# jketterl/digiham

Hardware: AMD Instinct MI355X
Metric: concurrent 48 kS/s DMR channels sustained end-to-end (rrc_filter->gfsk_demodulator->dmr_decoder) (higher is better)
Workload: dtype f32; 1 GPU; 16384 DMR channels/GPU x 3.96 s (190080 samples) of 48 kS/s FM-discriminator audio, full chain rrc(wide)->gfsk(10)->dmr_decoder incl. BPTC(196,96) (BASELINE con; channels_per_gpu=16384, total_channels=16384

## Files before the change

digiham_amd/csrc/dsp_core.hpp:

```cpp
#pragma once

#include "dh_portable.hpp"
#include "wave_ops.hpp"

#define DH_VARIANCE_SYMBOLS 100
#define DH_VOLUME_RB_SIZE 100
#define DH_FTILE 1024
#define DH_FIR_L 16
#define DH_PF_N 5
#define DH_PF_SINK 512
#define DH_MAX_NZ 160
#define DH_MAX_SPS 40
DH_HD uint32_t dh_history(uint32_t sps) { return DH_VARIANCE_SYMBOLS * (sps > 10u ? sps : 10u) + 152u; }
DH_HD uint32_t dh_tail_max(uint32_t sps) { return 256u + dh_history(sps); }
#define DH_STATE_HDR 32

enum { DH_ST_K = 0, DH_ST_OFF = 1, DH_ST_TAIL = 2, DH_ST_NSYM = 3, DH_ST_ORDERED = 4, DH_ST_BLOCKS = 5,
       DH_ST_P0 = 6,
       DH_ST_CUR_START = 7, DH_ST_CUR_OFF = 8, DH_ST_PREV_START = 9, DH_ST_PREV_OFF = 10,
       DH_ST_BLOCK_FLAGS = 11,
       DH_ST_E_CUR = 12, DH_ST_E_PREV = 13, DH_ST_E_COUNT = 14, DH_ST_E_BLOCK = 15,
       DH_ST_UNCERTAIN = 16, DH_ST_EXACT_RUNS = 17, DH_ST_EXACT_BLOCKS = 18,
       DH_ST_PART = 19,
       DH_ST_DIAG = 20 };
// ... 297 lines not shown
        float acc = 0.0f;
        for (int p = 0; p < NZ + 16; p++) acc = __builtin_fmaf(xs[DH_XPAD(b16 + (uint32_t) p)], tapsf[p - n], acc);
        acc16[4 * T + r] = acc;
    }
}
#endif

#define DH_EXACT_BATCH 2
#define DH_F16_KSTEPS_OF(nz) (((nz) + 16 + 31) / 32)
#define DH_F16_MAX_KSTEPS DH_F16_KSTEPS_OF(DH_MAX_NZ)
#define DH_F16_HALVES_OF(nz) (1008 + 32 * DH_F16_KSTEPS_OF(nz))
#define DH_F16_H2_OFFSET_OF(nz) (DH_F16_HALVES_OF(nz) / 2)
#define DH_F16_ROW_BLOCK(m) (2u * ((uint32_t) (m) & 3u) + (((uint32_t) (m) >> 2) & 1u) + 8u * ((uint32_t) (m) >> 3))
#define DH_F16_OUT(T, r, g, n) (256u * (uint32_t) (T) + 128u * ((uint32_t) (g) >> 1) + 32u * (uint32_t) (r) + 16u * ((uint32_t) (g) & 1u) + (uint32_t) (n))

struct DhF16Taps {
    uint32_t frag[2 * DH_F16_MAX_KSTEPS][DH_WAVE][4];
    uint32_t ksteps;
    double l1, l1_g1, l1_g2, sum_delta;
};
inline void dh_f16_tap_fragments(const float* taps_half, uint32_t nz, DhF16Taps& F) {
    uint16_t g1[DH_MAX_NZ + 1], g2[DH_MAX_NZ + 1];
    F.l1 = F.l1_g1 = F.l1_g2 = F.sum_delta = 0.0;
    for (uint32_t i = 0; i <= nz; i++) {
        const float c = taps_half[i <= nz / 2 ? i : nz - i];
        g1[i] = dh_f16_bits(c);
        const double r = (double) c - (double) dh_f16_value(g1[i]);
        g2[i] = dh_f16_bits((float) (r * 2048.0));
        const double v2 = (double) dh_f16_value(g2[i]);
        const double delta = r - v2 / 2048.0;
        F.l1 += c < 0 ? -(double) c : (double) c; F.l1_g1 += __builtin_fabs((double) dh_f16_value(g1[i]));
        F.l1_g2 += __builtin_fabs(v2); F.sum_delta += __builtin_fabs(delta);
    }
    const int KS = (int) DH_F16_KSTEPS_OF(nz);
    F.ksteps = (uint32_t) KS;
    for (int f = 0; f < 2 * KS; f++) for (int lane = 0; lane < DH_WAVE; lane++) for (int d = 0; d < 4; d++) {
        const int n = lane & 15, q = lane >> 4, s = f % KS;
        uint32_t w = 0;
        for (int hh = 0; hh < 2; hh++) {
            const int t = 32 * s + 8 * q + 2 * d + hh - n;
            const uint16_t v = (t >= 0 && t <= (int) nz) ? (f < KS ? g1[t] : g2[t]) : 0;
            w |= (uint32_t) v << (16 * hh);
        }
        F.frag[f][lane][d] = w;
    }
}
inline float dh_f16_error_coefficient(const DhF16Taps& F, uint32_t nz, double gain) {
    const double u = 5.9604644775390625e-08;
    const double ks = (double) F.ksteps, nref = 2.0 + (double) nz;
    const double kl1 = (nref + 0.01) * F.l1 + 1.0001 * F.l1 + 41.0 * ks * F.l1_g1 * (1.0 + 1.0 / 2048.0) + 82.0 * ks / 2048.0 * (F.l1_g2 + 0.5 * F.l1_g1)
                     + 2.0 * (0.5 * F.l1_g2 / 4194304.0 + F.sum_delta * (1.0 + 1.0 / 4096.0) + u * F.l1) / u + 3.1 * F.l1;
    const double coef = 1.44 * kl1 * u / (gain < 0 ? -gain : gain) * 1.0001;
    float f = (float) coef;
    if ((double) f < coef) { union { float f; uint32_t u; } b; b.f = f; b.u++; f = b.f; }
    return f;
}

#if DH_ON_GPU
template <int NZ>
__device__ __forceinline__ void dh_fir_f16(const float* hw, const dh_u4 (&G)[2 * DH_F16_KSTEPS_OF(NZ)], int lane, float k1, float k2, float* out16) {
    constexpr int DH_F16_KSTEPS = DH_F16_KSTEPS_OF(NZ), DH_F16_FRAGS = 2 * DH_F16_KSTEPS, DH_F16_H2_OFFSET = DH_F16_H2_OFFSET_OF(NZ);
    const int m = lane & 15, q = lane >> 4;
    const char* base = reinterpret_cast<const char*>(hw) + 32 * (int) DH_F16_ROW_BLOCK(m) + 16 * q;
    dh_h8 g[DH_F16_FRAGS];
#pragma unroll
    for (int f = 0; f < DH_F16_FRAGS; f++) g[f] = __builtin_bit_cast(dh_h8, G[f]);
#pragma unroll
    for (int TT = 0; TT < 4; TT += 2) {
        dh_h8 a1[2][DH_F16_KSTEPS], a2[2][DH_F16_KSTEPS];
#pragma unroll
        for (int t = 0; t < 2; t++)
#pragma unroll
            for (int s = 0; s < DH_F16_KSTEPS; s++) a1[t][s] = *reinterpret_cast<const dh_h8*>(base + 512 * (TT + t) + 64 * s);
        dh_f32x4 mn[2] = { { 0.0f, 0.0f, 0.0f, 0.0f }, { 0.0f, 0.0f, 0.0f, 0.0f } }, sc[2] = { { 0.0f, 0.0f, 0.0f, 0.0f }, { 0.0f, 0.0f, 0.0f, 0.0f } };
#pragma unroll
        for (int s = 0; s < DH_F16_KSTEPS; s++) {
#pragma unroll
            for (int t = 0; t < 2; t++) sc[t] = __builtin_amdgcn_mfma_f32_16x16x32_f16(a1[t][s], g[DH_F16_KSTEPS + s], sc[t], 0, 0, 0);
#pragma unroll
            for (int t = 0; t < 2; t++) mn[t] = __builtin_amdgcn_mfma_f32_16x16x32_f16(a1[t][s], g[s], mn[t], 0, 0, 0);
#pragma unroll
            for (int t = 0; t < 2; t++) a2[t][s] = *reinterpret_cast<const dh_h8*>(base + 512 * (TT + t) + 64 * s + 4 * DH_F16_H2_OFFSET);
        }
#pragma unroll
        for (int s = 0; s < DH_F16_KSTEPS; s++)
#pragma unroll
            for (int t = 0; t < 2; t++) sc[t] = __builtin_amdgcn_mfma_f32_16x16x32_f16(a2[t][s], g[s], sc[t], 0, 0, 0);
#pragma unroll
        for (int t = 0; t < 2; t++)
#pragma unroll
            for (int r = 0; r < 4; r++) out16[4 * (TT + t) + r] = __builtin_fmaf(sc[t][r], k2, mn[t][r] * k1);
        __builtin_amdgcn_sched_group_barrier(0x100, 2 * DH_F16_KSTEPS, 0);
#pragma unroll
        for (int s = 0; s < DH_F16_KSTEPS; s++) { __builtin_amdgcn_sched_group_barrier(0x008, 4, 0); __builtin_amdgcn_sched_group_barrier(0x100, 2, 0); }
        __builtin_amdgcn_sched_group_barrier(0x008, 2 * DH_F16_KSTEPS, 0);
    }
}
#else
template <int NZ>
inline void dh_fir_f16(const float* hw, const uint32_t (*G)[DH_WAVE][4], int lane, float k1, float k2, float* out16) {
    constexpr int DH_F16_KSTEPS = DH_F16_KSTEPS_OF(NZ), DH_F16_H2_OFFSET = DH_F16_H2_OFFSET_OF(NZ);
    const uint16_t* h1 = reinterpret_cast<const uint16_t*>(hw);
    const uint16_t* h2 = reinterpret_cast<const uint16_t*>(hw + DH_F16_H2_OFFSET);
    const int n = lane & 15, g = lane >> 4;
    for (int T = 0; T < 4; T++) for (int r = 0; r < 4; r++) {
        const uint32_t o = DH_F16_OUT(T, r, g, n), b16 = o - (uint32_t) n;
        float mn = 0.0f, sc = 0.0f;
        for (int pass = 0; pass < 3; pass++)
            for (int s = 0; s < DH_F16_KSTEPS; s++) for (int qq = 0; qq < 4; qq++) for (int j = 0; j < 8; j++) {
                const int kk = 8 * qq + j;
                const uint32_t w = G[(pass == 1 ? DH_F16_KSTEPS : 0) + s][16 * qq + n][j >> 1];
                const float tap = dh_f16_value((uint16_t) (w >> (16 * (j & 1))));
                const uint16_t hv = (pass == 2 ? h2 : h1)[b16 + 32u * (uint32_t) s + (uint32_t) kk];
                if (pass == 0) mn = __builtin_fmaf(dh_f16_value(hv), tap, mn); else sc = __builtin_fmaf(dh_f16_value(hv), tap, sc);
            }
        out16[4 * T + r] = __builtin_fmaf(sc, k2, mn * k1);
    }
}
#endif

DH_HD float dh_virtual_sample(const float* tail, uint32_t tc, const float* in, uint32_t idx) {
    return idx < tc ? tail[idx] : in[idx - tc];
}

struct DhAgcPair { float mn0, mx0, mn1, mx1; };

#if DH_ON_GPU
__device__ __forceinline__ void dh_agc_scan(DhDspShared& S, uint32_t k0, uint32_t k1, DH_LANE_STRUCT_REF(DhAgcPair, agc)) {
    const int lane = dh_fresh_lane_id_();
    const uint32_t e0 = 2u * (uint32_t) lane, e1 = e0 + 1u;
    const float c0 = e0 < k0 ? S.vol_old[e0] : S.vol_new[e0];
// ... 754 lines not shown
}
template <int NZ> struct DhWindowGroups {
    static constexpr uint32_t GSTEP = NZ > 0 ? DH_XPAD(4u * DH_WAVE) : 4u * DH_WAVE;
    static constexpr uint32_t LAST_LANES = (DH_FTILE + NZ - 4u * DH_WAVE * (DH_PF_N - 1)) / 4u;
    static constexpr uint32_t STORE_LANES = (DH_F16_HALVES_OF(NZ) - 4u * DH_WAVE * (DH_PF_N - 1)) / 4u;
    static_assert((DH_FTILE + NZ) % 4u == 0 && (DH_FTILE + NZ) >= 4u * DH_WAVE * (DH_PF_N - 1) && LAST_LANES <= DH_WAVE, "four full groups + a partial one cover the window");
    static_assert(STORE_LANES >= LAST_LANES && STORE_LANES <= DH_WAVE, "the partial group covers the padded arrays");
};
#define DH_STORE_FIR_OUT(xf, lane, fo) do { \
        dh_f4a* dst_ = reinterpret_cast<dh_f4a*>((xf) + DH_FIR_L * (lane)); \
        _Pragma("unroll") for (int j_ = 0; j_ < DH_FIR_L / 4; j_++) { \
            dh_f4a v_; v_.x = DH_LA(fo, lane)[4 * j_]; v_.y = DH_LA(fo, lane)[4 * j_ + 1]; \
            v_.z = DH_LA(fo, lane)[4 * j_ + 2]; v_.w = DH_LA(fo, lane)[4 * j_ + 3]; \
            dst_[j_] = v_; \
        } } while (0)
template <int NZ>
DH_HD bool dh_stage_f16(const DhDspParams& P, DhDspShared& S, DH_LANE_ARRAY(dh_f4, (&varr), DH_PF_N), uint32_t have, float& e_out, float& k1_out, float& k2_out) {
    constexpr uint32_t LAST_LANES = DhWindowGroups<NZ>::LAST_LANES, STORE_LANES = DhWindowGroups<NZ>::STORE_LANES;
    DH_LANE_ARRAY(float, xm, 1);
    DH_FOR_LANES_FRESH(lane) {
        const uint32_t l4 = 4u * (uint32_t) lane;
        if (DH_UNLIKELY(have < DH_FTILE + NZ)) {
#pragma unroll
            for (int r = 0; r < DH_PF_N; r++) {
                const uint32_t e = l4 + 4u * DH_WAVE * (uint32_t) r;
                DH_LA(varr, lane)[r] = dh_zero_beyond(DH_LA(varr, lane)[r], e, have);
            }
        }
        const float mx = dh_max_abs_groups(DH_LA(varr, lane));
        DH_LA(xm, lane)[0] = mx;
    }
    const float xmax = DH_WAVE_MAX(xm);
    float scale = 1.0f;
    if (xmax == 0.0f) { e_out = 0.0f; k1_out = P.inv_gain; }
    else if (xmax >= DH_BOUND_XMAX_LO && xmax <= DH_BOUND_XMAX_HI) {
        union { float f; uint32_t u; } b; b.f = xmax;
        const uint32_t ex = b.u >> 23;
        b.u = (253u - ex) << 23; scale = b.f;
        b.u = (ex + 1u) << 23; k1_out = P.inv_gain * b.f;
        e_out = P.err_coef_f16 * xmax;
    } else return false;
    k2_out = k1_out * 0.00048828125f;
    DH_FOR_LANES_FRESH(lane) {
        const bool in_last = (uint32_t) lane < LAST_LANES, in_store = (uint32_t) lane < STORE_LANES;
        if (STORE_LANES > LAST_LANES && !in_last) { dh_f4 z; z.x = 0.0f; z.y = 0.0f; z.z = 0.0f; z.w = 0.0f; DH_LA(varr, lane)[DH_PF_N - 1] = z; }
        dh_h4* d1 = reinterpret_cast<dh_h4*>(S.xf) + lane;
        dh_h4* d2 = reinterpret_cast<dh_h4*>(S.xf + DH_F16_H2_OFFSET_OF(NZ)) + lane;
#pragma unroll
        for (int r = 0; r < DH_PF_N; r++) {
            dh_h4 a, b;
            dh_f16_split4(DH_LA(varr, lane)[r], scale, a, b);
            if (r < DH_PF_N - 1 || in_store) { dh_h4_store(d1 + DH_WAVE * r, a); dh_h4_store(d2 + DH_WAVE * r, b); }
        }
    }
    return true;
}

template <int NZ, bool PF_REG>
DH_HD void dh_issue_next_window(DhDspShared& S, const float* const& in, const uint32_t& tc, const uint32_t& p_next, const bool& pf_plain, const bool& pf_reg, DH_LANE_ARRAY(dh_f4, (&pfr), PF_REG ? DH_PF_N : 1)) {
    (void) S; (void) pfr;
    if (DH_LIKELY(pf_reg)) {
        constexpr uint32_t LAST_LANES = DhWindowGroups<NZ>::LAST_LANES;
        const float* src = in + (p_next - tc);
        DH_FOR_LANES_FRESH(lane) {
            const float* lsrc = src + 4u * (uint32_t) lane;
            const bool in_last = (uint32_t) lane < LAST_LANES;
// ... 3 lines not shown
            else (void) in_last;
        }
    } else {
        if (pf_plain) dh_l2_touch_lines(in + (p_next - tc), DH_FTILE + NZ, S.xf + DH_PF_SINK);
    }
}

#define DH_TAIL_GROUPS 8
#define DH_RING_GROUPS 16

template <int NZ, bool FAST, int SPS, int LV = 0, int KEEPF = 0>
DH_HD void dh_rrc_demod_channel(const DhDspParams& P, uint32_t ch, DhDspShared& S, uint32_t part_lo = 0, uint32_t part_hi = 0xFFFFFFFFu, uint32_t sym_base = 0) {
    static_assert(SPS == 0 || SPS == 10 || SPS == 20 || SPS == 40, "0 = run-time samples per symbol; 10 has its own window and timing code, 20 / 40 are the generic code with the constant folded in");
    constexpr bool BOUNDED = DhIsBounded<NZ, FAST, SPS>::value;
    constexpr bool MF16 = BOUNDED && (NZ == 80 || NZ == 160) && KEEPF != 2;
    DhBoundState* const BS = DH_BOUND_STATE(S);
    float* st = P.state + (size_t) ch * P.state_stride;
    uint32_t* sth = (uint32_t*) st;
    const uint32_t sps = SPS ? (uint32_t) SPS : P.sps;
    const uint32_t ev_lo = SPS == 10 ? 3u : SPS == 20 ? 7u : SPS == 40 ? 13u : P.lo, ev_hi = SPS == 10 ? 7u : SPS == 20 ? 13u : SPS == 40 ? 27u : P.hi;
    const float sps_rcp = 1.0f / (float) sps;
    float* tail = st + DH_ST_VAR + DH_VARIANCE_SYMBOLS * sps;
    const float* in = P.in + (size_t) ch * P.in_stride + part_lo;
    uint8_t* syms = P.syms + (size_t) ch * P.sym_stride;
    const float* in_end = P.in + (size_t) (P.n_channels - 1u) * P.in_stride + P.n;
    const ptrdiff_t in_room = (in_end - in) - (ptrdiff_t) (DH_FTILE + NZ);
    const uint32_t win_lim = dh_uniform(in_room < 0 ? 0u : in_room >= (ptrdiff_t) 0xFFFFFFFFu ? 0xFFFFFFFFu : (uint32_t) in_room + 1u);

    DH_PHASE_MARK_BEGIN();
    uint32_t k0 = sth[DH_ST_K];
// ... 147 lines not shown
                        }
                    }
                    if (BOUNDED) {
                        float mx = 0.0f;
#pragma unroll
                        for (int r = 0; r < DH_PF_N; r++) {
                            const dh_f4 w = DH_LA(v, lane)[r];
                            mx = dh_max3_abs(w.x, w.y, mx); mx = dh_max3_abs(w.z, w.w, mx);
                        }
                        DH_LA(xmax_lane, lane)[0] = mx;
                    }
                }
            }
            if (MF16 && !use_exact) {
                xmax_done = true;
                if (dh_stage_f16<NZ>(P, S, v, have, e_run, k1, k2)) f16_staged = true; else use_exact = true;
            }
            if (!f16_staged) {
                DH_FOR_LANES_FRESH(lane) {
                    const uint32_t l4 = 4u * (uint32_t) lane;
                    const bool in_last = (uint32_t) lane < LAST_LANES;
                    float* ldst = &S.xf[DH_XP(l4)];
                    dh_lds_store4_at<0>(ldst, DH_LA(v, lane)[0]); dh_lds_store4_at<GSTEP>(ldst, DH_LA(v, lane)[1]);
                    dh_lds_store4_at<2 * GSTEP>(ldst, DH_LA(v, lane)[2]); dh_lds_store4_at<3 * GSTEP>(ldst, DH_LA(v, lane)[3]);
                    static_assert(DH_PF_N == 5, "four full groups + a partial one");
                    if constexpr (LAST_LANES > 0) { if (in_last) dh_lds_store4_at<4 * GSTEP>(ldst, DH_LA(v, lane)[4]); }
                    dh_lds_stores_done();
                }
            }
        } else if (MF16 && !use_exact) {
            const uint32_t have = dh_min<uint32_t>(DH_FTILE + NZ, nv - p);
            DH_LANE_ARRAY(dh_f4, v, DH_PF_N);
            DH_FOR_LANES_FRESH(lane) {
#pragma unroll
                for (int r = 0; r < DH_PF_N; r++) {
                    const uint32_t e = 4u * (uint32_t) lane + 4u * DH_WAVE * (uint32_t) r;
                    dh_f4 w;
                    w.x = e + 0u < have ? dh_virtual_sample(tail, tc, in, p + e + 0u) : 0.0f;
                    w.y = e + 1u < have ? dh_virtual_sample(tail, tc, in, p + e + 1u) : 0.0f;
                    w.z = e + 2u < have ? dh_virtual_sample(tail, tc, in, p + e + 2u) : 0.0f;
                    w.w = e + 3u < have ? dh_virtual_sample(tail, tc, in, p + e + 3u) : 0.0f;
                    DH_LA(v, lane)[r] = w;
                }
            }
            xmax_done = true;
            if (dh_stage_f16<NZ>(P, S, v, have, e_run, k1, k2)) f16_staged = true;
            else {
                use_exact = true;
                dh_gather_window<NZ>(S, tail, tc, in, nv, p);
            }
        } else if (p >= tc) {
            use_exact = BOUNDED;
            const float* src = in + (p - tc);
            const uint32_t have = dh_min<uint32_t>(DH_FTILE + NZ, nv - p);
            DH_FOR_LANES_FRESH(lane) {
                for (uint32_t e = 4u * (uint32_t) lane; e < DH_FTILE + NZ; e += 4u * DH_WAVE) {
                    dh_f4 v;
                    if (e + 4u <= have) v = dh_load4_unaligned(src + e);
                    else {
                        v.x = e + 0u < have ? src[e + 0u] : 0.0f; v.y = e + 1u < have ? src[e + 1u] : 0.0f;
                        v.z = e + 2u < have ? src[e + 2u] : 0.0f; v.w = e + 3u < have ? src[e + 3u] : 0.0f;
                    }
                    dh_store4(&S.xf[DH_XP(e)], v);
                }
            }
        } else {
            use_exact = BOUNDED;
            dh_gather_window<NZ>(S, tail, tc, in, nv, p);
        }
        DH_BARRIER();
        if (BOUNDED && !use_exact && !xmax_done) {
            const float xmax = DH_WAVE_MAX(xmax_lane);
            if (xmax == 0.0f) e_run = 0.0f;
            else if (xmax >= DH_BOUND_XMAX_LO && xmax <= DH_BOUND_XMAX_HI) e_run = P.err_coef * xmax;
            else use_exact = true;
        }
        DH_PHASE_MARK(0);

        if (NZ > 0 && DH_STOP_AFTER >= 2) {
            DH_LANE_ARRAY(float, fo, DH_FIR_L);
            DH_COMPILER_FENCE();
            constexpr bool MFMA = NZ > 0 && NZ <= 80 && (BOUNDED || FAST) && !MF16;
            int mf_layout = 0;
            if (BOUNDED) {
                uint64_t vote_bad = 0;
                if (DH_LIKELY(!use_exact)) {
                    if constexpr (MF16) {
                        DH_FOR_LANES_FRESH(lane) {
                            float t = 0.0f;
                            dh_fir_f16<MF16 ? NZ : 80>(S.xf, tapfrag_regs, lane, k1, k2, DH_LA(fo, lane));
#pragma unroll
                            for (int j = 0; j < DH_FIR_L; j++) t = __builtin_fmaf(DH_LA(fo, lane)[j], 0.0f, t);
                            DH_BALLOT_ACC(vote_bad, !(t == 0.0f), lane);
                        }
                        mf_layout = 2;
                    } else if constexpr (MFMA) {
                        DH_FOR_LANES_FRESH(lane) {
                            bool bad = false;
                            float acc[DH_FIR_L];
                            dh_fir_mfma<MFMA ? NZ : 80>(S.tapsf, S.xf, lane, acc);
                            dh_fir_finish<true>(acc, P.gain, P.rgain, P.inv_gain, DH_LA(fo, lane), &bad);
                            DH_BALLOT_ACC(vote_bad, bad, lane);
                        }
                        mf_layout = 1;
                    } else static_assert(!BOUNDED, "every error-bounded kernel filters on the matrix cores (launch_plan.hpp instantiates none without MF16 or MFMA)");
                }
                if (DH_UNLIKELY(use_exact || vote_bad)) {
                    use_exact = true; e_run = 0.0f; BS->n_exact_runs++; mf_layout = 0;
// ... 101 lines not shown
        const bool block_done = (k0 + m == DH_VARIANCE_SYMBOLS);
        if (block_done && DH_STOP_AFTER >= 6) {
            new_off = dh_timing_decision<NZ, SPS, BOUNDED>(P, S, BS, V, sps, k0, e_blk);
        }

        DH_PHASE_MARK(5);
        DH_FOR_LANES_FRESH(lane) {
            const uint32_t ka = k0 + (uint32_t) lane, kb = ka + DH_WAVE, ke = k0 + m;
            const uint32_t ia = ka < ke ? ka : k0, ib = kb < ke ? kb : k0;
            const float va_ = S.vol_new[ia], vb_ = S.vol_new[ib];
            S.vol_old[ia] = va_;
            S.vol_old[ib] = vb_;
        }
        staged_p = 0xFFFFFFFFu;
        if (DH_LIKELY(pf_reg)) {
            if constexpr (PF_REG && MF16) { if (DH_LIKELY(dh_stage_f16<NZ>(P, S, pfr, pf_have, st_e_run, st_k1, st_k2))) staged_p = p_next; }
            else if constexpr (PF_PLAIN) {
                static_assert(!PF_PLAIN || (DH_FTILE == 4u * DH_WAVE * (DH_PF_N - 1)), "four full groups cover the window");
                DH_FOR_LANES_FRESH(lane) {
                    const uint32_t l4 = 4u * (uint32_t) lane;
                    float* ldst = &S.xf[l4];
#pragma unroll
                    for (int r = 0; r < DH_PF_N - 1; r++) {
                        dh_f4 w = DH_LA(pfr, lane)[PF_REG ? r : 0];
                        if (DH_UNLIKELY(pf_have < DH_FTILE)) w = dh_zero_beyond(w, l4 + 4u * DH_WAVE * (uint32_t) r, pf_have);
                        dh_store4(ldst + 4 * DH_WAVE * r, w);
                    }
                }
                staged_p = p_next;
            }
        }
// ... 180 lines not shown
```

digiham_amd/csrc/engine_impl.hpp:

```cpp
#pragma once

#include <stdlib.h>
#include <string.h>
#include <new>
#include <vector>

#include "../../include/digiham_amd.h"
#include "dsp_core.hpp"
#include "decoder_core.hpp"
#include "kernels_core.hpp"
#include "fec_tables.hpp"
#include "rrc_taps.h"

namespace dh {

struct Layout {
    uint32_t B, max_samples, sps, nz, lo, hi;
    int rrc, demod, proto;
    uint32_t flags;
    uint32_t sym_cap, out_cap, ev_cap;
    size_t sym_stride, state_words;
    bool fused;
    int fused_keep;
};
// ... 129 lines not shown
        if (!ok) return DH_ENOMEM;
        configure(c.rrc_gain);
        if (L.proto) {
            DhFecTables* host = new (std::nothrow) DhFecTables;
            if (!host) return DH_ENOMEM;
            build_fec_tables(*host);
            rc = be.upload(tables, host, sizeof(DhFecTables));
            be.sync();
            delete host;
            if (rc) return rc;
        }
        if (L.rrc == DH_RRC_CUSTOM && (be.upload(custom_taps, c.rrc_taps, sizeof(float) * (L.nz + 1)) || be.sync())) return DH_EDEVICE;
        if (tapfrag) {
            DhF16Taps* F = new (std::nothrow) DhF16Taps;
            if (!F) return DH_ENOMEM;
            dh_f16_tap_fragments(dsp.taps, L.nz, *F);
            dsp.err_coef_f16 = dh_f16_error_coefficient(*F, L.nz, dsp.gain);
            rc = be.upload(tapfrag, F->frag, sizeof(F->frag)) || be.sync();
            delete F;
            if (rc) return DH_EDEVICE;
        }
        return reset();
    }

    void configure(double custom_gain) {
        fast = (L.flags & DH_FLAG_FAST_FIR) != 0;
        const bool own_rrc = L.rrc && !L.fused;
        if (L.rrc == DH_RRC_CUSTOM) {
            gen.out = filtered; gen.out_stride = L.max_samples; gen.hist = rrc_hist; gen.taps = custom_taps;
            gen.n_channels = L.B; gen.nz = L.nz; gen.gain = custom_gain;
        } else if (own_rrc) {
// ... 183 lines not shown
```

digiham_amd/csrc/wave_ops.hpp:

```cpp
#pragma once

#include "dh_portable.hpp"

#define DH_FLT_MAX 3.402823466e+38f
#define DH_DBL_MAX 1.7976931348623157e+308
#define DH_FLT_MIN 1.175494351e-38f

#if DH_ON_GPU
typedef float dh_f2 __attribute__((ext_vector_type(2)));
typedef float dh_v4f __attribute__((ext_vector_type(4)));
typedef float dh_f32x4 __attribute__((ext_vector_type(4)));
typedef _Float16 dh_h8 __attribute__((ext_vector_type(8)));
typedef _Float16 dh_h4 __attribute__((ext_vector_type(4)));
typedef uint32_t dh_u4 __attribute__((ext_vector_type(4)));
#else
struct dh_f2 { float x, y; };
typedef uint16_t dh_h4[4];
#endif
struct __attribute__((aligned(4))) dh_f4 { float x, y, z, w; };
struct alignas(16) dh_f4a { float x, y, z, w; };
DH_HD dh_f4 dh_load4_unaligned(const float* p) { dh_f4 v; __builtin_memcpy(&v, p, sizeof(v)); return v; }
DH_HD void dh_store4(float* q, const dh_f4& v) { q[0] = v.x; q[1] = v.y; q[2] = v.z; q[3] = v.w; }
DH_HD void dh_store4_unaligned(float* q, const dh_f4& v) { __builtin_memcpy(q, &v, sizeof(v)); }

// ... 62 lines not shown
#else
inline dh_f2 dh_div_const2(dh_f2 x, float d, float r) { return dh_f2_make(dh_div_const(x.x, d, r), dh_div_const(x.y, d, r)); }
#endif

DH_HD float dh_sqrt_upper(float x) {
    const float a = x > 1e-30f ? x : 1e-30f;
    return DH_GPU_ELSE(__builtin_amdgcn_sqrtf(a), __builtin_sqrtf(a)) * 1.00000095367431640625f;
}

DH_HD float dh_fmin_(float a, float b) { return b < a ? b : a; }
DH_HD float dh_fmax_(float a, float b) { return b > a ? b : a; }
#if DH_ON_GPU
__device__ __forceinline__ float dh_vmin(float a, float b) { float r; asm("v_min_f32 %0, %1, %2" : "=v"(r) : "v"(a), "v"(b)); return r; }
__device__ __forceinline__ float dh_vmax(float a, float b) { float r; asm("v_max_f32 %0, %1, %2" : "=v"(r) : "v"(a), "v"(b)); return r; }
__device__ __forceinline__ float dh_min3_abs(float a, float b, float c) { float r; asm("v_min3_f32 %0, |%1|, |%2|, |%3|" : "=v"(r) : "v"(a), "v"(b), "v"(c)); return r; }
__device__ __forceinline__ float dh_max3_abs(float a, float b, float c) { float r; asm("v_max3_f32 %0, |%1|, |%2|, %3" : "=v"(r) : "v"(a), "v"(b), "v"(c)); return r; }
#else
inline float dh_vmin(float a, float b) { return __builtin_fminf(a, b); }
inline float dh_vmax(float a, float b) { return __builtin_fmaxf(a, b); }
inline float dh_min3_abs(float a, float b, float c) { return __builtin_fminf(__builtin_fminf(__builtin_fabsf(a), __builtin_fabsf(b)), __builtin_fabsf(c)); }
inline float dh_max3_abs(float a, float b, float c) { return __builtin_fmaxf(c, __builtin_fmaxf(__builtin_fabsf(a), __builtin_fabsf(b))); }
#endif
template <int N> DH_HD float dh_max_abs_groups(const dh_f4 (&w)[N]) {
#if DH_ON_GPU
    static_assert(N == 5, "five groups of four");
    float mx;
    const dh_f4 w0 = w[0], w1 = w[1], w2 = w[2], w3 = w[3], w4 = w[4];
    asm("v_max3_f32 %0, |%1|, |%2|, 0\n\tv_max3_f32 %0, |%3|, |%4|, %0\n\tv_max3_f32 %0, |%5|, |%6|, %0\n\tv_max3_f32 %0, |%7|, |%8|, %0\n\t"
        "v_max3_f32 %0, |%9|, |%10|, %0\n\tv_max3_f32 %0, |%11|, |%12|, %0\n\tv_max3_f32 %0, |%13|, |%14|, %0\n\tv_max3_f32 %0, |%15|, |%16|, %0\n\t"
        "v_max3_f32 %0, |%17|, |%18|, %0\n\tv_max3_f32 %0, |%19|, |%20|, %0"
        : "=&v"(mx) : "v"(w0.x), "v"(w0.y), "v"(w0.z), "v"(w0.w), "v"(w1.x), "v"(w1.y), "v"(w1.z), "v"(w1.w), "v"(w2.x), "v"(w2.y), "v"(w2.z), "v"(w2.w),
                      "v"(w3.x), "v"(w3.y), "v"(w3.z), "v"(w3.w), "v"(w4.x), "v"(w4.y), "v"(w4.z), "v"(w4.w));
    return mx;
#else
    float mx = 0.0f;
    for (int r = 0; r < N; r++) { mx = dh_max3_abs(w[r].x, w[r].y, mx); mx = dh_max3_abs(w[r].z, w[r].w, mx); }
    return mx;
#endif
}

DH_HD uint16_t dh_f16_bits(float f) {
    union { float f; uint32_t u; } v; v.f = f;
    const uint32_t sign = (v.u >> 16) & 0x8000u, a = v.u & 0x7FFFFFFFu;
    if (a >= 0x7F800000u) return (uint16_t) (sign | (a > 0x7F800000u ? 0x7E00u : 0x7C00u));
    if (a >= 0x477FF000u) return (uint16_t) (sign | 0x7C00u);
// ... 16 lines not shown
DH_HD void dh_f16_split4(const dh_f4& v, float scale, dh_h4& h1, dh_h4& h2) {
    const float x[4] = { v.x, v.y, v.z, v.w };
#pragma unroll
    for (int i = 0; i < 4; i++) {
        const float xs = x[i] * scale;
#if DH_ON_GPU
        const _Float16 a = (_Float16) xs;
        const float r = xs - (float) a;
        h1[i] = a; h2[i] = (_Float16) (r * 2048.0f);
#else
        h1[i] = dh_f16_bits(xs);
        const float r = xs - dh_f16_value(h1[i]);
        h2[i] = dh_f16_bits(r * 2048.0f);
#endif
    }
}
DH_HD void dh_h4_store(dh_h4* dst, const dh_h4& v) { __builtin_memcpy(dst, &v, sizeof(dh_h4)); }

#if DH_ON_GPU
template <int O0, int O1> __device__ __forceinline__ dh_f2 dh_lds_read2(uint32_t addr) {
    static_assert(O0 < 256 && O1 < 256, "ds_read2_b32 offsets are 8-bit dword counts");
    dh_f2 v;
    asm volatile("ds_read2_b32 %0, %1 offset0:%2 offset1:%3" : "=v"(v) : "v"(addr), "n"(O0), "n"(O1) : "memory");
    return v;
}
template <int OFF_BYTES> __device__ __forceinline__ dh_f2 dh_lds_read_b64(uint32_t addr) {
    dh_f2 v;
    asm volatile("ds_read_b64 %0, %1 offset:%2" : "=v"(v) : "v"(addr), "n"(OFF_BYTES) : "memory");
    return v;
}
// ... 107 lines not shown
    asm volatile("s_nop 4\n\tv_mov_b32_dpp %0, %4 wave_shr:1 row_mask:0xf bank_mask:0xf\n\tv_mov_b32_dpp %1, %5 wave_shr:1 row_mask:0xf bank_mask:0xf\n\t"
                 "v_mov_b32_dpp %2, %6 wave_shr:1 row_mask:0xf bank_mask:0xf\n\tv_mov_b32_dpp %3, %7 wave_shr:1 row_mask:0xf bank_mask:0xf\n\ts_nop 1"
                 : "+v"(a), "+v"(b), "+v"(c), "+v"(d) : "v"(va), "v"(vb), "v"(vc), "v"(vd));
}

__device__ __forceinline__ float dh_wave_max(float v) {
#define DH_MAX_STEP(ctrl) "s_nop 1\n\tv_max_f32_dpp %0, %0, %0 " ctrl "\n\t"
    asm volatile("s_nop 4\n\t"
                 DH_MAX_STEP("row_shr:1 row_mask:0xf bank_mask:0xf") DH_MAX_STEP("row_shr:2 row_mask:0xf bank_mask:0xf")
                 DH_MAX_STEP("row_shr:4 row_mask:0xf bank_mask:0xf") DH_MAX_STEP("row_shr:8 row_mask:0xf bank_mask:0xf")
                 DH_MAX_STEP("row_bcast:15 row_mask:0xa bank_mask:0xf") DH_MAX_STEP("row_bcast:31 row_mask:0xc bank_mask:0xf")
                 "s_nop 1" : "+v"(v));
#undef DH_MAX_STEP
    return __int_as_float(__builtin_amdgcn_readlane(__float_as_int(v), 63));
}
__device__ __forceinline__ float dh_row_min_to_lane15(float v) {
    asm volatile("s_nop 4\n\tv_min_f32_dpp %0, %0, %0 row_shr:1 row_mask:0xf bank_mask:0xf\n\t"
                 "s_nop 1\n\tv_min_f32_dpp %0, %0, %0 row_shr:2 row_mask:0xf bank_mask:0xf\n\t"
                 "s_nop 1\n\tv_min_f32_dpp %0, %0, %0 row_shr:4 row_mask:0xf bank_mask:0xf\n\t"
                 "s_nop 1\n\tv_min_f32_dpp %0, %0, %0 row_shr:8 row_mask:0xf bank_mask:0xf\n\ts_nop 1"
                 : "+v"(v));
    return __int_as_float(__builtin_amdgcn_readlane(__float_as_int(v), 15));
}
#else
inline float dh_wave_max_lanes(const float (&a)[DH_WAVE][1]) {
    float m = 0.0f;
    for (int l = 0; l < DH_WAVE; l++) m = __builtin_fmaxf(m, a[l][0]);
    return m;
}
inline float dh_wave_min_lanes(const float (&a)[DH_WAVE][1], int lanes) {
    float m = DH_FLT_MAX;
    for (int l = 0; l < lanes; l++) m = dh_fmin_(m, a[l][0]);
    return m;
}
#endif
#if DH_ON_GPU
#define DH_WAVE_MAX(a) dh_wave_max((a)[0])
#define DH_WAVE_MIN(a) (-dh_wave_max(-(a)[0]))
#define DH_ROW0_MIN(a) dh_row_min_to_lane15((a)[0])
#else
#define DH_WAVE_MAX(a) dh_wave_max_lanes(a)
#define DH_WAVE_MIN(a) dh_wave_min_lanes(a, DH_WAVE)
#define DH_ROW0_MIN(a) dh_wave_min_lanes(a, 16)
#endif

DH_HD void dh_row_sum5_pair(DH_LANE_ARRAY(float, (&gs), 1), DH_LANE_ARRAY(float, (&gq), 1)) {
#if DH_ON_GPU
    float s = gs[0], q = gq[0], t1, t2, u1, u2;
    asm volatile("s_nop 4\n\t"
                 "v_add_f32_dpp %0, %4, %4 row_shr:1 row_mask:0xf bank_mask:0xf bound_ctrl:0\n\t"
                 "v_add_f32_dpp %2, %5, %5 row_shr:1 row_mask:0xf bank_mask:0xf bound_ctrl:0\n\t"
                 "s_nop 0\n\t"
                 "v_add_f32_dpp %1, %0, %0 row_shr:2 row_mask:0xf bank_mask:0xf bound_ctrl:0\n\t"
                 "v_add_f32_dpp %3, %2, %2 row_shr:2 row_mask:0xf bank_mask:0xf bound_ctrl:0\n\t"
                 "v_add_f32_dpp %1, %4, %1 row_shr:4 row_mask:0xf bank_mask:0xf bound_ctrl:0\n\t"
                 "v_add_f32_dpp %3, %5, %3 row_shr:4 row_mask:0xf bank_mask:0xf bound_ctrl:0"
// ... 14 lines not shown
```

Before: 14.01 million channels.

## Fold f16 split-FIR into one MFMA accumulator chain for NZ=80

For the 80-tap f16 MFMA FIR path, the high-part taps are pre-scaled by 2048 so the main and correction products accumulate in a single f32 accumulator instead of two. This removes the final fma combine and uses a simpler input split without the 2048 scaling. The per-tile NaN vote is dropped for NZ=80, and NaN detection moves into the xmax reduction via v_maximum3 and an unsigned-integer wave max. The error bound is recomputed for the one-chain case, and setup now fails if the scaled taps overflow f16. Trade-off: fewer VALU ops and accumulator registers, but a longer serial MFMA dependency chain.

```diff
diff --git a/digiham_amd/csrc/dsp_core.hpp b/digiham_amd/csrc/dsp_core.hpp
--- a/digiham_amd/csrc/dsp_core.hpp
+++ b/digiham_amd/csrc/dsp_core.hpp
@@ -335,14 +335,19 @@
 #define DH_F16_ROW_BLOCK(m) (2u * ((uint32_t) (m) & 3u) + (((uint32_t) (m) >> 2) & 1u) + 8u * ((uint32_t) (m) >> 3))
 #define DH_F16_OUT(T, r, g, n) (256u * (uint32_t) (T) + 128u * ((uint32_t) (g) >> 1) + 32u * (uint32_t) (r) + 16u * ((uint32_t) (g) & 1u) + (uint32_t) (n))
 
+constexpr bool dh_f16_one_chain(uint32_t nz, int keepf) { return nz == 80 && !keepf; }
+
 struct DhF16Taps {
     uint32_t frag[2 * DH_F16_MAX_KSTEPS][DH_WAVE][4];
     uint32_t ksteps;
+    bool one_chain;
     double l1, l1_g1, l1_g2, sum_delta;
 };
-inline void dh_f16_tap_fragments(const float* taps_half, uint32_t nz, DhF16Taps& F) {
+inline bool dh_f16_tap_fragments(const float* taps_half, uint32_t nz, bool one_chain, DhF16Taps& F) {
     uint16_t g1[DH_MAX_NZ + 1], g2[DH_MAX_NZ + 1];
     F.l1 = F.l1_g1 = F.l1_g2 = F.sum_delta = 0.0;
+    F.one_chain = one_chain;
+    bool ok = true;
     for (uint32_t i = 0; i <= nz; i++) {
         const float c = taps_half[i <= nz / 2 ? i : nz - i];
         g1[i] = dh_f16_bits(c);
@@ -352,6 +357,12 @@
         const double delta = r - v2 / 2048.0;
         F.l1 += c < 0 ? -(double) c : (double) c; F.l1_g1 += __builtin_fabs((double) dh_f16_value(g1[i]));
         F.l1_g2 += __builtin_fabs(v2); F.sum_delta += __builtin_fabs(delta);
+        if (one_chain) {
+            const float v1 = dh_f16_value(g1[i]);
+            g1[i] = dh_f16_bits(v1 * 2048.0f);
+            const float s1 = dh_f16_value(g1[i]);
+            if (!(s1 == v1 * 2048.0f) || (g1[i] & 0x7C00u) == 0x7C00u) ok = false;
+        }
     }
     const int KS = (int) DH_F16_KSTEPS_OF(nz);
     F.ksteps = (uint32_t) KS;
@@ -365,12 +376,15 @@
         }
         F.frag[f][lane][d] = w;
     }
+    return ok;
 }
 inline float dh_f16_error_coefficient(const DhF16Taps& F, uint32_t nz, double gain) {
     const double u = 5.9604644775390625e-08;
     const double ks = (double) F.ksteps, nref = 2.0 + (double) nz;
-    const double kl1 = (nref + 0.01) * F.l1 + 1.0001 * F.l1 + 41.0 * ks * F.l1_g1 * (1.0 + 1.0 / 2048.0) + 82.0 * ks / 2048.0 * (F.l1_g2 + 0.5 * F.l1_g1)
-                     + 2.0 * (0.5 * F.l1_g2 / 4194304.0 + F.sum_delta * (1.0 + 1.0 / 4096.0) + u * F.l1) / u + 3.1 * F.l1;
+    const double mfma = F.one_chain ? 82.0 * ks * F.l1_g1 * (1.0 + 1.0 / 2048.0) + 41.0 * ks / 2048.0 * (3.0 * F.l1_g2 * (1.0 + 1.0 / 2048.0) + F.l1_g1)
+                                    : 41.0 * ks * F.l1_g1 * (1.0 + 1.0 / 2048.0) + 82.0 * ks / 2048.0 * (F.l1_g2 + 0.5 * F.l1_g1);
+    const double kl1 = (nref + 0.01) * F.l1 + 1.0001 * F.l1 + mfma
+                     + 2.0 * (0.5 * F.l1_g2 / 4194304.0 + F.sum_delta * (1.0 + 1.0 / 4096.0) + u * F.l1) / u + (F.one_chain ? 2.1 : 3.1) * F.l1;
     const double coef = 1.44 * kl1 * u / (gain < 0 ? -gain : gain) * 1.0001;
     float f = (float) coef;
     if ((double) f < coef) { union { float f; uint32_t u; } b; b.f = f; b.u++; f = b.f; }
@@ -378,7 +392,7 @@
 }
 
 #if DH_ON_GPU
-template <int NZ>
+template <int NZ, bool ONE>
 __device__ __forceinline__ void dh_fir_f16(const float* hw, const dh_u4 (&G)[2 * DH_F16_KSTEPS_OF(NZ)], int lane, float k1, float k2, float* out16) {
     constexpr int DH_F16_KSTEPS = DH_F16_KSTEPS_OF(NZ), DH_F16_FRAGS = 2 * DH_F16_KSTEPS, DH_F16_H2_OFFSET = DH_F16_H2_OFFSET_OF(NZ);
     const int m = lane & 15, q = lane >> 4;
@@ -393,32 +407,61 @@
         for (int t = 0; t < 2; t++)
 #pragma unroll
             for (int s = 0; s < DH_F16_KSTEPS; s++) a1[t][s] = *reinterpret_cast<const dh_h8*>(base + 512 * (TT + t) + 64 * s);
-        dh_f32x4 mn[2] = { { 0.0f, 0.0f, 0.0f, 0.0f }, { 0.0f, 0.0f, 0.0f, 0.0f } }, sc[2] = { { 0.0f, 0.0f, 0.0f, 0.0f }, { 0.0f, 0.0f, 0.0f, 0.0f } };
-#pragma unroll
-        for (int s = 0; s < DH_F16_KSTEPS; s++) {
-#pragma unroll
-            for (int t = 0; t < 2; t++) sc[t] = __builtin_amdgcn_mfma_f32_16x16x32_f16(a1[t][s], g[DH_F16_KSTEPS + s], sc[t], 0, 0, 0);
-#pragma unroll
-            for (int t = 0; t < 2; t++) mn[t] = __builtin_amdgcn_mfma_f32_16x16x32_f16(a1[t][s], g[s], mn[t], 0, 0, 0);
-#pragma unroll
-            for (int t = 0; t < 2; t++) a2[t][s] = *reinterpret_cast<const dh_h8*>(base + 512 * (TT + t) + 64 * s + 4 * DH_F16_H2_OFFSET);
-        }
-#pragma unroll
-        for (int s = 0; s < DH_F16_KSTEPS; s++)
-#pragma unroll
-            for (int t = 0; t < 2; t++) sc[t] = __builtin_amdgcn_mfma_f32_16x16x32_f16(a2[t][s], g[s], sc[t], 0, 0, 0);
-#pragma unroll
-        for (int t = 0; t < 2; t++)
-#pragma unroll
-            for (int r = 0; r < 4; r++) out16[4 * (TT + t) + r] = __builtin_fmaf(sc[t][r], k2, mn[t][r] * k1);
-        __builtin_amdgcn_sched_group_barrier(0x100, 2 * DH_F16_KSTEPS, 0);
-#pragma unroll
-        for (int s = 0; s < DH_F16_KSTEPS; s++) { __builtin_amdgcn_sched_group_barrier(0x008, 4, 0); __builtin_amdgcn_sched_group_barrier(0x100, 2, 0); }
-        __builtin_amdgcn_sched_group_barrier(0x008, 2 * DH_F16_KSTEPS, 0);
+        if constexpr (ONE) {
+            dh_f32x4 acc[2] = { { 0.0f, 0.0f, 0.0f, 0.0f }, { 0.0f, 0.0f, 0.0f, 0.0f } };
+#pragma unroll
+            for (int s = 0; s < DH_F16_KSTEPS; s++)
+#pragma unroll
+                for (int t = 0; t < 2; t++) acc[t] = __builtin_amdgcn_mfma_f32_16x16x32_f16(a1[t][s], g[DH_F16_KSTEPS + s], acc[t], 0, 0, 0);
+#pragma unroll
+            for (int s = 0; s < DH_F16_KSTEPS; s++) {
+#pragma unroll
+                for (int t = 0; t < 2; t++) acc[t] = __builtin_amdgcn_mfma_f32_16x16x32_f16(a1[t][s], g[s], acc[t], 0, 0, 0);
+#pragma unroll
+                for (int t = 0; t < 2; t++) a2[t][s] = *reinterpret_cast<const dh_h8*>(base + 512 * (TT + t) + 64 * s + 4 * DH_F16_H2_OFFSET);
+            }
+#pragma unroll
+            for (int s = 0; s < DH_F16_KSTEPS; s++)
+#pragma unroll
+                for (int t = 0; t < 2; t++) acc[t] = __builtin_amdgcn_mfma_f32_16x16x32_f16(a2[t][s], g[s], acc[t], 0, 0, 0);
+#pragma unroll
+            for (int t = 0; t < 2; t++)
+#pragma unroll
+                for (int r = 0; r < 4; r++) out16[4 * (TT + t) + r] = acc[t][r] * k1;
+            __builtin_amdgcn_sched_group_barrier(0x100, 2 * DH_F16_KSTEPS, 0);
+            __builtin_amdgcn_sched_group_barrier(0x008, 2 * DH_F16_KSTEPS, 0);
+#pragma unroll
+            for (int s = 0; s < DH_F16_KSTEPS; s++) { __builtin_amdgcn_sched_group_barrier(0x008, 2, 0); __builtin_amdgcn_sched_group_barrier(0x100, 2, 0); }
+            __builtin_amdgcn_sched_group_barrier(0x008, 2 * DH_F16_KSTEPS, 0);
+            (void) k2;
+        } else {
+            dh_f32x4 mn[2] = { { 0.0f, 0.0f, 0.0f, 0.0f }, { 0.0f, 0.0f, 0.0f, 0.0f } }, sc[2] = { { 0.0f, 0.0f, 0.0f, 0.0f }, { 0.0f, 0.0f, 0.0f, 0.0f } };
+#pragma unroll
+            for (int s = 0; s < DH_F16_KSTEPS; s++) {
+#pragma unroll
+                for (int t = 0; t < 2; t++) sc[t] = __builtin_amdgcn_mfma_f32_16x16x32_f16(a1[t][s], g[DH_F16_KSTEPS + s], sc[t], 0, 0, 0);
+#pragma unroll
+                for (int t = 0; t < 2; t++) mn[t] = __builtin_amdgcn_mfma_f32_16x16x32_f16(a1[t][s], g[s], mn[t], 0, 0, 0);
+#pragma unroll
+                for (int t = 0; t < 2; t++) a2[t][s] = *reinterpret_cast<const dh_h8*>(base + 512 * (TT + t) + 64 * s + 4 * DH_F16_H2_OFFSET);
+            }
+#pragma unroll
+            for (int s = 0; s < DH_F16_KSTEPS; s++)
+#pragma unroll
+                for (int t = 0; t < 2; t++) sc[t] = __builtin_amdgcn_mfma_f32_16x16x32_f16(a2[t][s], g[s], sc[t], 0, 0, 0);
+#pragma unroll
+            for (int t = 0; t < 2; t++)
+#pragma unroll
+                for (int r = 0; r < 4; r++) out16[4 * (TT + t) + r] = __builtin_fmaf(sc[t][r], k2, mn[t][r] * k1);
+            __builtin_amdgcn_sched_group_barrier(0x100, 2 * DH_F16_KSTEPS, 0);
+#pragma unroll
+            for (int s = 0; s < DH_F16_KSTEPS; s++) { __builtin_amdgcn_sched_group_barrier(0x008, 4, 0); __builtin_amdgcn_sched_group_barrier(0x100, 2, 0); }
+            __builtin_amdgcn_sched_group_barrier(0x008, 2 * DH_F16_KSTEPS, 0);
+        }
     }
 }
 #else
-template <int NZ>
+template <int NZ, bool ONE>
 inline void dh_fir_f16(const float* hw, const uint32_t (*G)[DH_WAVE][4], int lane, float k1, float k2, float* out16) {
     constexpr int DH_F16_KSTEPS = DH_F16_KSTEPS_OF(NZ), DH_F16_H2_OFFSET = DH_F16_H2_OFFSET_OF(NZ);
     const uint16_t* h1 = reinterpret_cast<const uint16_t*>(hw);
@@ -427,15 +470,17 @@
     for (int T = 0; T < 4; T++) for (int r = 0; r < 4; r++) {
         const uint32_t o = DH_F16_OUT(T, r, g, n), b16 = o - (uint32_t) n;
         float mn = 0.0f, sc = 0.0f;
-        for (int pass = 0; pass < 3; pass++)
+        for (int i = 0; i < 3; i++) {
+            const int pass = ONE ? (i == 0 ? 1 : i == 1 ? 0 : 2) : i;
             for (int s = 0; s < DH_F16_KSTEPS; s++) for (int qq = 0; qq < 4; qq++) for (int j = 0; j < 8; j++) {
                 const int kk = 8 * qq + j;
                 const uint32_t w = G[(pass == 1 ? DH_F16_KSTEPS : 0) + s][16 * qq + n][j >> 1];
                 const float tap = dh_f16_value((uint16_t) (w >> (16 * (j & 1))));
                 const uint16_t hv = (pass == 2 ? h2 : h1)[b16 + 32u * (uint32_t) s + (uint32_t) kk];
-                if (pass == 0) mn = __builtin_fmaf(dh_f16_value(hv), tap, mn); else sc = __builtin_fmaf(dh_f16_value(hv), tap, sc);
-            }
-        out16[4 * T + r] = __builtin_fmaf(sc, k2, mn * k1);
+                if (pass == 0 && !ONE) mn = __builtin_fmaf(dh_f16_value(hv), tap, mn); else sc = __builtin_fmaf(dh_f16_value(hv), tap, sc);
+            }
+        }
+        out16[4 * T + r] = ONE ? sc * k1 : __builtin_fmaf(sc, k2, mn * k1);
     }
 }
 #endif
@@ -1220,7 +1265,7 @@
             v_.z = DH_LA(fo, lane)[4 * j_ + 2]; v_.w = DH_LA(fo, lane)[4 * j_ + 3]; \
             dst_[j_] = v_; \
         } } while (0)
-template <int NZ>
+template <int NZ, bool ONE>
 DH_HD bool dh_stage_f16(const DhDspParams& P, DhDspShared& S, DH_LANE_ARRAY(dh_f4, (&varr), DH_PF_N), uint32_t have, float& e_out, float& k1_out, float& k2_out) {
     constexpr uint32_t LAST_LANES = DhWindowGroups<NZ>::LAST_LANES, STORE_LANES = DhWindowGroups<NZ>::STORE_LANES;
     DH_LANE_ARRAY(float, xm, 1);
@@ -1236,17 +1281,17 @@
         const float mx = dh_max_abs_groups(DH_LA(varr, lane));
         DH_LA(xm, lane)[0] = mx;
     }
-    const float xmax = DH_WAVE_MAX(xm);
+    const float xmax = DH_WAVE_MAX_NAN(xm);
     float scale = 1.0f;
     if (xmax == 0.0f) { e_out = 0.0f; k1_out = P.inv_gain; }
     else if (xmax >= DH_BOUND_XMAX_LO && xmax <= DH_BOUND_XMAX_HI) {
         union { float f; uint32_t u; } b; b.f = xmax;
         const uint32_t ex = b.u >> 23;
         b.u = (253u - ex) << 23; scale = b.f;
-        b.u = (ex + 1u) << 23; k1_out = P.inv_gain * b.f;
+        b.u = (ex + 1u - (ONE ? 11u : 0u)) << 23; k1_out = P.inv_gain * b.f;
         e_out = P.err_coef_f16 * xmax;
     } else return false;
-    k2_out = k1_out * 0.00048828125f;
+    k2_out = ONE ? 0.0f : k1_out * 0.00048828125f;
     DH_FOR_LANES_FRESH(lane) {
         const bool in_last = (uint32_t) lane < LAST_LANES, in_store = (uint32_t) lane < STORE_LANES;
         if (STORE_LANES > LAST_LANES && !in_last) { dh_f4 z; z.x = 0.0f; z.y = 0.0f; z.z = 0.0f; z.w = 0.0f; DH_LA(varr, lane)[DH_PF_N - 1] = z; }
@@ -1255,7 +1300,7 @@
 #pragma unroll
         for (int r = 0; r < DH_PF_N; r++) {
             dh_h4 a, b;
-            dh_f16_split4(DH_LA(varr, lane)[r], scale, a, b);
+            if constexpr (ONE) dh_f16_split4_plain(DH_LA(varr, lane)[r], scale, a, b); else dh_f16_split4(DH_LA(varr, lane)[r], scale, a, b);
             if (r < DH_PF_N - 1 || in_store) { dh_h4_store(d1 + DH_WAVE * r, a); dh_h4_store(d2 + DH_WAVE * r, b); }
         }
     }
@@ -1289,6 +1334,8 @@
     static_assert(SPS == 0 || SPS == 10 || SPS == 20 || SPS == 40, "0 = run-time samples per symbol; 10 has its own window and timing code, 20 / 40 are the generic code with the constant folded in");
     constexpr bool BOUNDED = DhIsBounded<NZ, FAST, SPS>::value;
     constexpr bool MF16 = BOUNDED && (NZ == 80 || NZ == 160) && KEEPF != 2;
+    constexpr bool ONE_CHAIN = dh_f16_one_chain(NZ, KEEPF);
+    constexpr bool F16_KEEPS_VOTE = MF16 && NZ == 160;
     DhBoundState* const BS = DH_BOUND_STATE(S);
     float* st = P.state + (size_t) ch * P.state_stride;
     uint32_t* sth = (uint32_t*) st;
@@ -1466,7 +1513,7 @@
             }
             if (MF16 && !use_exact) {
                 xmax_done = true;
-                if (dh_stage_f16<NZ>(P, S, v, have, e_run, k1, k2)) f16_staged = true; else use_exact = true;
+                if (dh_stage_f16<NZ, ONE_CHAIN>(P, S, v, have, e_run, k1, k2)) f16_staged = true; else use_exact = true;
             }
             if (!f16_staged) {
                 DH_FOR_LANES_FRESH(lane) {
@@ -1496,7 +1543,7 @@
                 }
             }
             xmax_done = true;
-            if (dh_stage_f16<NZ>(P, S, v, have, e_run, k1, k2)) f16_staged = true;
+            if (dh_stage_f16<NZ, ONE_CHAIN>(P, S, v, have, e_run, k1, k2)) f16_staged = true;
             else {
                 use_exact = true;
                 dh_gather_window<NZ>(S, tail, tc, in, nv, p);
@@ -1522,7 +1569,7 @@
         }
         DH_BARRIER();
         if (BOUNDED && !use_exact && !xmax_done) {
-            const float xmax = DH_WAVE_MAX(xmax_lane);
+            const float xmax = DH_WAVE_MAX_NAN(xmax_lane);
             if (xmax == 0.0f) e_run = 0.0f;
             else if (xmax >= DH_BOUND_XMAX_LO && xmax <= DH_BOUND_XMAX_HI) e_run = P.err_coef * xmax;
             else use_exact = true;
@@ -1539,11 +1586,13 @@
                 if (DH_LIKELY(!use_exact)) {
                     if constexpr (MF16) {
                         DH_FOR_LANES_FRESH(lane) {
-                            float t = 0.0f;
-                            dh_fir_f16<MF16 ? NZ : 80>(S.xf, tapfrag_regs, lane, k1, k2, DH_LA(fo, lane));
-#pragma unroll
-                            for (int j = 0; j < DH_FIR_L; j++) t = __builtin_fmaf(DH_LA(fo, lane)[j], 0.0f, t);
-                            DH_BALLOT_ACC(vote_bad, !(t == 0.0f), lane);
+                            dh_fir_f16<MF16 ? NZ : 80, ONE_CHAIN>(S.xf, tapfrag_regs, lane, k1, k2, DH_LA(fo, lane));
+                            if constexpr (F16_KEEPS_VOTE) {
+                                float t = 0.0f;
+#pragma unroll
+                                for (int j = 0; j < DH_FIR_L; j++) t = __builtin_fmaf(DH_LA(fo, lane)[j], 0.0f, t);
+                                DH_BALLOT_ACC(vote_bad, !(t == 0.0f), lane);
+                            }
                         }
                         mf_layout = 2;
                     } else if constexpr (MFMA) {
@@ -1675,7 +1724,7 @@
         }
         staged_p = 0xFFFFFFFFu;
         if (DH_LIKELY(pf_reg)) {
-            if constexpr (PF_REG && MF16) { if (DH_LIKELY(dh_stage_f16<NZ>(P, S, pfr, pf_have, st_e_run, st_k1, st_k2))) staged_p = p_next; }
+            if constexpr (PF_REG && MF16) { if (DH_LIKELY((dh_stage_f16<NZ, ONE_CHAIN>(P, S, pfr, pf_have, st_e_run, st_k1, st_k2)))) staged_p = p_next; }
             else if constexpr (PF_PLAIN) {
                 static_assert(!PF_PLAIN || (DH_FTILE == 4u * DH_WAVE * (DH_PF_N - 1)), "four full groups cover the window");
                 DH_FOR_LANES_FRESH(lane) {
diff --git a/digiham_amd/csrc/engine_impl.hpp b/digiham_amd/csrc/engine_impl.hpp
--- a/digiham_amd/csrc/engine_impl.hpp
+++ b/digiham_amd/csrc/engine_impl.hpp
@@ -167,7 +167,7 @@
         if (tapfrag) {
             DhF16Taps* F = new (std::nothrow) DhF16Taps;
             if (!F) return DH_ENOMEM;
-            dh_f16_tap_fragments(dsp.taps, L.nz, *F);
+            if (!dh_f16_tap_fragments(dsp.taps, L.nz, dh_f16_one_chain(L.nz, L.fused_keep), *F)) { delete F; return DH_EINVAL; }
             dsp.err_coef_f16 = dh_f16_error_coefficient(*F, L.nz, dsp.gain);
             rc = be.upload(tapfrag, F->frag, sizeof(F->frag)) || be.sync();
             delete F;
diff --git a/digiham_amd/csrc/wave_ops.hpp b/digiham_amd/csrc/wave_ops.hpp
--- a/digiham_amd/csrc/wave_ops.hpp
+++ b/digiham_amd/csrc/wave_ops.hpp
@@ -100,21 +100,24 @@
 __device__ __forceinline__ float dh_vmin(float a, float b) { float r; asm("v_min_f32 %0, %1, %2" : "=v"(r) : "v"(a), "v"(b)); return r; }
 __device__ __forceinline__ float dh_vmax(float a, float b) { float r; asm("v_max_f32 %0, %1, %2" : "=v"(r) : "v"(a), "v"(b)); return r; }
 __device__ __forceinline__ float dh_min3_abs(float a, float b, float c) { float r; asm("v_min3_f32 %0, |%1|, |%2|, |%3|" : "=v"(r) : "v"(a), "v"(b), "v"(c)); return r; }
-__device__ __forceinline__ float dh_max3_abs(float a, float b, float c) { float r; asm("v_max3_f32 %0, |%1|, |%2|, %3" : "=v"(r) : "v"(a), "v"(b), "v"(c)); return r; }
+__device__ __forceinline__ float dh_max3_abs(float a, float b, float c) { float r; asm("v_maximum3_f32 %0, |%1|, |%2|, %3" : "=v"(r) : "v"(a), "v"(b), "v"(c)); return r; }
 #else
 inline float dh_vmin(float a, float b) { return __builtin_fminf(a, b); }
 inline float dh_vmax(float a, float b) { return __builtin_fmaxf(a, b); }
 inline float dh_min3_abs(float a, float b, float c) { return __builtin_fminf(__builtin_fminf(__builtin_fabsf(a), __builtin_fabsf(b)), __builtin_fabsf(c)); }
-inline float dh_max3_abs(float a, float b, float c) { return __builtin_fmaxf(c, __builtin_fmaxf(__builtin_fabsf(a), __builtin_fabsf(b))); }
+inline float dh_max3_abs(float a, float b, float c) {
+    if (a != a || b != b || c != c) return __builtin_nanf("");
+    return __builtin_fmaxf(c, __builtin_fmaxf(__builtin_fabsf(a), __builtin_fabsf(b)));
+}
 #endif
 template <int N> DH_HD float dh_max_abs_groups(const dh_f4 (&w)[N]) {
 #if DH_ON_GPU
     static_assert(N == 5, "five groups of four");
     float mx;
     const dh_f4 w0 = w[0], w1 = w[1], w2 = w[2], w3 = w[3], w4 = w[4];
-    asm("v_max3_f32 %0, |%1|, |%2|, 0\n\tv_max3_f32 %0, |%3|, |%4|, %0\n\tv_max3_f32 %0, |%5|, |%6|, %0\n\tv_max3_f32 %0, |%7|, |%8|, %0\n\t"
-        "v_max3_f32 %0, |%9|, |%10|, %0\n\tv_max3_f32 %0, |%11|, |%12|, %0\n\tv_max3_f32 %0, |%13|, |%14|, %0\n\tv_max3_f32 %0, |%15|, |%16|, %0\n\t"
-        "v_max3_f32 %0, |%17|, |%18|, %0\n\tv_max3_f32 %0, |%19|, |%20|, %0"
+    asm("v_maximum3_f32 %0, |%1|, |%2|, 0\n\tv_maximum3_f32 %0, |%3|, |%4|, %0\n\tv_maximum3_f32 %0, |%5|, |%6|, %0\n\tv_maximum3_f32 %0, |%7|, |%8|, %0\n\t"
+        "v_maximum3_f32 %0, |%9|, |%10|, %0\n\tv_maximum3_f32 %0, |%11|, |%12|, %0\n\tv_maximum3_f32 %0, |%13|, |%14|, %0\n\tv_maximum3_f32 %0, |%15|, |%16|, %0\n\t"
+        "v_maximum3_f32 %0, |%17|, |%18|, %0\n\tv_maximum3_f32 %0, |%19|, |%20|, %0"
         : "=&v"(mx) : "v"(w0.x), "v"(w0.y), "v"(w0.z), "v"(w0.w), "v"(w1.x), "v"(w1.y), "v"(w1.z), "v"(w1.w), "v"(w2.x), "v"(w2.y), "v"(w2.z), "v"(w2.w),
                       "v"(w3.x), "v"(w3.y), "v"(w3.z), "v"(w3.w), "v"(w4.x), "v"(w4.y), "v"(w4.z), "v"(w4.w));
     return mx;
@@ -161,6 +164,27 @@
         h2[i] = dh_f16_bits(r * 2048.0f);
 #endif
     }
+}
+DH_HD void dh_f16_split4_plain(const dh_f4& v, float scale, dh_h4& h1, dh_h4& h2) {
+#if DH_ON_GPU
+    dh_v4f xs; xs.x = v.x; xs.y = v.y; xs.z = v.z; xs.w = v.w;
+    xs = xs * scale;
+    const dh_h4 a = __builtin_convertvector(xs, dh_h4);
+    const dh_v4f af = __builtin_convertvector(a, dh_v4f);
+    const dh_f2 x01 = xs.xy, x23 = xs.zw, a01 = af.xy, a23 = af.zw;
+    dh_f2 r01, r23;
+    asm("v_pk_add_f32 %0, %1, %2 neg_lo:[0,1] neg_hi:[0,1]" : "=v"(r01) : "v"(x01), "v"(a01));
+    asm("v_pk_add_f32 %0, %1, %2 neg_lo:[0,1] neg_hi:[0,1]" : "=v"(r23) : "v"(x23), "v"(a23));
+    dh_v4f r; r.xy = r01; r.zw = r23;
+    h1 = a; h2 = __builtin_convertvector(r, dh_h4);
+#else
+    const float x[4] = { v.x, v.y, v.z, v.w };
+    for (int i = 0; i < 4; i++) {
+        const float xs = x[i] * scale;
+        h1[i] = dh_f16_bits(xs);
+        h2[i] = dh_f16_bits(xs - dh_f16_value(h1[i]));
+    }
+#endif
 }
 DH_HD void dh_h4_store(dh_h4* dst, const dh_h4& v) { __builtin_memcpy(dst, &v, sizeof(dh_h4)); }
 
@@ -298,6 +322,17 @@
 #undef DH_MAX_STEP
     return __int_as_float(__builtin_amdgcn_readlane(__float_as_int(v), 63));
 }
+__device__ __forceinline__ float dh_wave_max_nan(float f) {
+    uint32_t v = __float_as_uint(f);
+#define DH_MAX_STEP(ctrl) "s_nop 1\n\tv_max_u32_dpp %0, %0, %0 " ctrl "\n\t"
+    asm volatile("s_nop 4\n\t"
+                 DH_MAX_STEP("row_shr:1 row_mask:0xf bank_mask:0xf") DH_MAX_STEP("row_shr:2 row_mask:0xf bank_mask:0xf")
+                 DH_MAX_STEP("row_shr:4 row_mask:0xf bank_mask:0xf") DH_MAX_STEP("row_shr:8 row_mask:0xf bank_mask:0xf")
+                 DH_MAX_STEP("row_bcast:15 row_mask:0xa bank_mask:0xf") DH_MAX_STEP("row_bcast:31 row_mask:0xc bank_mask:0xf")
+                 "s_nop 1" : "+v"(v));
+#undef DH_MAX_STEP
+    return __int_as_float(__builtin_amdgcn_readlane((int) v, 63));
+}
 __device__ __forceinline__ float dh_row_min_to_lane15(float v) {
     asm volatile("s_nop 4\n\tv_min_f32_dpp %0, %0, %0 row_shr:1 row_mask:0xf bank_mask:0xf\n\t"
                  "s_nop 1\n\tv_min_f32_dpp %0, %0, %0 row_shr:2 row_mask:0xf bank_mask:0xf\n\t"
@@ -312,6 +347,12 @@
     for (int l = 0; l < DH_WAVE; l++) m = __builtin_fmaxf(m, a[l][0]);
     return m;
 }
+inline float dh_wave_max_nan_lanes(const float (&a)[DH_WAVE][1]) {
+    uint32_t m = 0;
+    for (int l = 0; l < DH_WAVE; l++) { union { float f; uint32_t u; } b; b.f = a[l][0]; if (b.u > m) m = b.u; }
+    union { float f; uint32_t u; } r; r.u = m;
+    return r.f;
+}
 inline float dh_wave_min_lanes(const float (&a)[DH_WAVE][1], int lanes) {
     float m = DH_FLT_MAX;
     for (int l = 0; l < lanes; l++) m = dh_fmin_(m, a[l][0]);
@@ -320,10 +361,12 @@
 #endif
 #if DH_ON_GPU
 #define DH_WAVE_MAX(a) dh_wave_max((a)[0])
+#define DH_WAVE_MAX_NAN(a) dh_wave_max_nan((a)[0])
 #define DH_WAVE_MIN(a) (-dh_wave_max(-(a)[0]))
 #define DH_ROW0_MIN(a) dh_row_min_to_lane15((a)[0])
 #else
 #define DH_WAVE_MAX(a) dh_wave_max_lanes(a)
+#define DH_WAVE_MAX_NAN(a) dh_wave_max_nan_lanes(a)
 #define DH_WAVE_MIN(a) dh_wave_min_lanes(a, DH_WAVE)
 #define DH_ROW0_MIN(a) dh_wave_min_lanes(a, 16)
 #endif
```

Result: faster. 14.39 million channels (median of 6 runs) (+2.7%).
